# arkworks-rs/ripp

Measured on AMD Instinct MI355X. Metric: SIPP prover pairing-products/sec at n=2^20 BLS12-381, higher is better.
Workload: dtype u32

## Files before the change

### ripp_amd/csrc/bls12_381/tower.hpp

```cpp
#pragma once
#include "fp.hpp"
#include "fp_inv.hpp"

namespace ripp {

struct Fp2 {
    Fp c0, c1;
    RIPP_HD static Fp2 zero() { return {Fp::zero(), Fp::zero()}; }
    RIPP_HD static Fp2 one() { return {Fp::one(), Fp::zero()}; }
    RIPP_HD bool is_zero() const { return c0.is_zero() && c1.is_zero(); }
    RIPP_HD bool operator==(const Fp2& o) const { return c0 == o.c0 && c1 == o.c1; }
};
RIPP_HD Fp2 add(const Fp2& a, const Fp2& b) { return {add(a.c0, b.c0), add(a.c1, b.c1)}; }
RIPP_HD Fp2 sub(const Fp2& a, const Fp2& b) { return {sub(a.c0, b.c0), sub(a.c1, b.c1)}; }
RIPP_HD Fp2 neg(const Fp2& a) { return {neg(a.c0), neg(a.c1)}; }
RIPP_HD Fp2 dbl(const Fp2& a) { return {dbl(a.c0), dbl(a.c1)}; }
RIPP_HD Fp2 conj(const Fp2& a) { return {a.c0, neg(a.c1)}; }
#if defined(RIPP_BLS12_377)
RIPP_HD Fp mul5(const Fp& a) { const Fp t = dbl(dbl(a)); return add(t, a); }
RIPP_MID Fp2 mul(const Fp2& a, const Fp2& b) {
    const Fp t0 = fmul(a.c0, b.c0), t1 = fmul(a.c1, b.c1);
    const Fp m = fmul(add(a.c0, a.c1), add(b.c0, b.c1));
    return {sub(t0, mul5(t1)), sub(sub(m, t0), t1)};
}
RIPP_MID Fp2 sqr(const Fp2& a) {
    const Fp m = fmul(a.c0, a.c1);
    return {add(fmul(add(a.c0, a.c1), sub(a.c0, mul5(a.c1))), dbl(dbl(m))), dbl(m)};
}
RIPP_MID Fp2 mul_fp(const Fp2& a, const Fp& s) { return {fmul(a.c0, s), fmul(a.c1, s)}; }
RIPP_HD Fp2 mul_xi(const Fp2& a) { return {neg(mul5(a.c1)), a.c0}; }
RIPP_MID Fp2 inv(const Fp2& a) {
    const Fp n = finv(add(fsqr(a.c0), mul5(fsqr(a.c1))));
    return {fmul(a.c0, n), neg(fmul(a.c1, n))};
}
#else
RIPP_MID Fp2 mul(const Fp2& a, const Fp2& b) {
    const Fp t0 = fmul(a.c0, b.c0), t1 = fmul(a.c1, b.c1);
    const Fp m = fmul(add(a.c0, a.c1), add(b.c0, b.c1));
    return {sub(t0, t1), sub(sub(m, t0), t1)};
}
RIPP_MID Fp2 sqr(const Fp2& a) {
    const Fp m = fmul(a.c0, a.c1);
    return {fmul(add(a.c0, a.c1), sub(a.c0, a.c1)), dbl(m)};
}
RIPP_MID Fp2 mul_fp(const Fp2& a, const Fp& s) { return {fmul(a.c0, s), fmul(a.c1, s)}; }
RIPP_HD Fp2 mul_xi(const Fp2& a) { return {sub(a.c0, a.c1), add(a.c0, a.c1)}; }
RIPP_MID Fp2 inv(const Fp2& a) {
    const Fp n = finv(add(fsqr(a.c0), fsqr(a.c1)));
    return {fmul(a.c0, n), neg(fmul(a.c1, n))};
}
#endif

RIPP_HD Fp2 finv(const Fp2& a) { return inv(a); }
#if defined(__HIP_DEVICE_COMPILE__) && !defined(RIPP_NO_FP2_LAZY) && defined(RIPP_BLS12_377)
RIPP_MID Fp2 fmul(const Fp2& a, const Fp2& b) { return {fmul2_add(a.c0, b.c0, neg(mul5(a.c1)), b.c1), fmul2_add(a.c0, b.c1, a.c1, b.c0)}; }
#elif defined(__HIP_DEVICE_COMPILE__) && !defined(RIPP_NO_FP2_LAZY)
RIPP_MID Fp2 fmul(const Fp2& a, const Fp2& b) { return {fmul2_add(a.c0, b.c0, neg(a.c1), b.c1), fmul2_add(a.c0, b.c1, a.c1, b.c0)}; }
#else
RIPP_HD Fp2 fmul(const Fp2& a, const Fp2& b) { return mul(a, b); }
#endif
RIPP_HD Fp2 fsqr(const Fp2& a) { return sqr(a); }

struct Fp6 {
    Fp2 c0, c1, c2;
    RIPP_HD static Fp6 zero() { return {Fp2::zero(), Fp2::zero(), Fp2::zero()}; }
    RIPP_HD static Fp6 one() { return {Fp2::one(), Fp2::zero(), Fp2::zero()}; }
    RIPP_HD bool operator==(const Fp6& o) const { return c0 == o.c0 && c1 == o.c1 && c2 == o.c2; }
};
RIPP_HD Fp6 add(const Fp6& a, const Fp6& b) { return {add(a.c0, b.c0), add(a.c1, b.c1), add(a.c2, b.c2)}; }
RIPP_HD Fp6 sub(const Fp6& a, const Fp6& b) { return {sub(a.c0, b.c0), sub(a.c1, b.c1), sub(a.c2, b.c2)}; }
RIPP_HD Fp6 neg(const Fp6& a) { return {neg(a.c0), neg(a.c1), neg(a.c2)}; }
RIPP_HD Fp6 mul_v(const Fp6& a) { return {mul_xi(a.c2), a.c0, a.c1}; }
RIPP_MID Fp6 mul(const Fp6& a, const Fp6& b) {
    const Fp2 v0 = mul(a.c0, b.c0), v1 = mul(a.c1, b.c1), v2 = mul(a.c2, b.c2);
    const Fp2 t0 = add(mul_xi(sub(sub(mul(add(a.c1, a.c2), add(b.c1, b.c2)), v1), v2)), v0);
    const Fp2 t1 = add(sub(sub(mul(add(a.c0, a.c1), add(b.c0, b.c1)), v0), v1), mul_xi(v2));
    const Fp2 t2 = add(sub(sub(mul(add(a.c0, a.c2), add(b.c0, b.c2)), v0), v2), v1);
    return {t0, t1, t2};
}
RIPP_MID Fp6 mul_by_01(const Fp6& a, const Fp2& b0, const Fp2& b1) {
    const Fp2 v0 = mul(a.c0, b0), v1 = mul(a.c1, b1);
    const Fp2 t0 = add(mul_xi(sub(mul(add(a.c1, a.c2), b1), v1)), v0);
    const Fp2 t1 = sub(sub(mul(add(a.c0, a.c1), add(b0, b1)), v0), v1);
    const Fp2 t2 = add(sub(mul(add(a.c0, a.c2), b0), v0), v1);
    return {t0, t1, t2};
}
RIPP_MID Fp6 mul_by_1(const Fp6& a, const Fp2& b1) { return {mul_xi(mul(a.c2, b1)), mul(a.c0, b1), mul(a.c1, b1)}; }
RIPP_FN Fp6 inv(const Fp6& a) {
    const Fp2 A = sub(sqr(a.c0), mul_xi(mul(a.c1, a.c2)));
    const Fp2 B = sub(mul_xi(sqr(a.c2)), mul(a.c0, a.c1));
    const Fp2 C = sub(sqr(a.c1), mul(a.c0, a.c2));
    const Fp2 F = inv(add(mul_xi(add(mul(a.c2, B), mul(a.c1, C))), mul(a.c0, A)));
    return {mul(A, F), mul(B, F), mul(C, F)};
}

struct Fp12 {
    Fp6 c0, c1;
    RIPP_HD static Fp12 one() { return {Fp6::one(), Fp6::zero()}; }
    RIPP_HD bool operator==(const Fp12& o) const { return c0 == o.c0 && c1 == o.c1; }
};
RIPP_HD Fp12 conj(const Fp12& a) { return {a.c0, neg(a.c1)}; }
RIPP_MID Fp12 mul(const Fp12& a, const Fp12& b) {
    const Fp6 v0 = mul(a.c0, b.c0), v1 = mul(a.c1, b.c1);
    const Fp6 x = sub(sub(mul(add(a.c0, a.c1), add(b.c0, b.c1)), v0), v1);
    return {add(v0, mul_v(v1)), x};
}
RIPP_MID Fp12 sqr(const Fp12& a) {
    const Fp6 v0 = mul(a.c0, a.c1);
    const Fp6 s = sub(sub(mul(add(a.c0, a.c1), add(a.c0, mul_v(a.c1))), v0), mul_v(v0));
    return {s, add(v0, v0)};
}
RIPP_MID Fp12 mul_by_014(const Fp12& f, const Fp2& c0, const Fp2& c1, const Fp2& c4) {
    const Fp6 aa = mul_by_01(f.c0, c0, c1);
    const Fp6 bb = mul_by_1(f.c1, c4);
    const Fp6 s = sub(sub(mul_by_01(add(f.c1, f.c0), c0, add(c1, c4)), aa), bb);
    return {add(mul_v(bb), aa), s};
}
RIPP_MID Fp12 mul_by_034(const Fp12& f, const Fp2& c0, const Fp2& d0, const Fp2& d1) {
    const Fp6 a = {mul(f.c0.c0, c0), mul(f.c0.c1, c0), mul(f.c0.c2, c0)};
    const Fp6 b = mul_by_01(f.c1, d0, d1);
    const Fp6 e = sub(sub(mul_by_01(add(f.c0, f.c1), add(c0, d0), d1), a), b);
    return {add(a, mul_v(b)), e};
}
RIPP_FN Fp12 inv(const Fp12& a) {
    const Fp6 t = inv(sub(mul(a.c0, a.c0), mul_v(mul(a.c1, a.c1))));
    return {mul(a.c0, t), neg(mul(a.c1, t))};
}

RIPP_FN Fp12 frobenius(const Fp12& a, int k) {
    Fp2 g[6] = {a.c0.c0, a.c1.c0, a.c0.c1, a.c1.c1, a.c0.c2, a.c1.c2};
    for (int i = 0; i < 6; ++i) {
        constexpr uint32_t T[3][6][2][12] = {
            {{RIPP_FROB1_W0_C0, RIPP_FROB1_W0_C1}, {RIPP_FROB1_W1_C0, RIPP_FROB1_W1_C1}, {RIPP_FROB1_W2_C0, RIPP_FROB1_W2_C1},
             {RIPP_FROB1_W3_C0, RIPP_FROB1_W3_C1}, {RIPP_FROB1_W4_C0, RIPP_FROB1_W4_C1}, {RIPP_FROB1_W5_C0, RIPP_FROB1_W5_C1}},
            {{RIPP_FROB2_W0_C0, RIPP_FROB2_W0_C1}, {RIPP_FROB2_W1_C0, RIPP_FROB2_W1_C1}, {RIPP_FROB2_W2_C0, RIPP_FROB2_W2_C1},
             {RIPP_FROB2_W3_C0, RIPP_FROB2_W3_C1}, {RIPP_FROB2_W4_C0, RIPP_FROB2_W4_C1}, {RIPP_FROB2_W5_C0, RIPP_FROB2_W5_C1}},
            {{RIPP_FROB3_W0_C0, RIPP_FROB3_W0_C1}, {RIPP_FROB3_W1_C0, RIPP_FROB3_W1_C1}, {RIPP_FROB3_W2_C0, RIPP_FROB3_W2_C1},
             {RIPP_FROB3_W3_C0, RIPP_FROB3_W3_C1}, {RIPP_FROB3_W4_C0, RIPP_FROB3_W4_C1}, {RIPP_FROB3_W5_C0, RIPP_FROB3_W5_C1}}};
        Fp2 coef;
        for (int j = 0; j < 12; ++j) { coef.c0.l[j] = T[k - 1][i][0][j]; coef.c1.l[j] = T[k - 1][i][1][j]; }
        g[i] = mul((k & 1) ? conj(g[i]) : g[i], coef);
    }
    return {{g[0], g[2], g[4]}, {g[1], g[3], g[5]}};
}

RIPP_HD void fp4_sqr(Fp2& o0, Fp2& o1, const Fp2& x, const Fp2& y) {
    const Fp2 t0 = sqr(x), t1 = sqr(y);
    o1 = sub(sub(sqr(add(x, y)), t0), t1);
    o0 = add(t0, mul_xi(t1));
}
RIPP_FN Fp12 cyclotomic_sqr(const Fp12& a) {
    const Fp2 &z0 = a.c0.c0, &z4 = a.c0.c1, &z3 = a.c0.c2, &z2 = a.c1.c0, &z1 = a.c1.c1, &z5 = a.c1.c2;
    Fp2 t0, t1, t2, t3, t4, t5;
    fp4_sqr(t0, t1, z0, z1); fp4_sqr(t2, t3, z2, z3); fp4_sqr(t4, t5, z4, z5);
    const Fp2 xt5 = mul_xi(t5);
    Fp12 o;
    o.c0.c0 = add(dbl(sub(t0, z0)), t0);
    o.c1.c1 = add(dbl(add(t1, z1)), t1);
    o.c1.c0 = add(dbl(add(xt5, z2)), xt5);
    o.c0.c2 = add(dbl(sub(t4, z3)), t4);
    o.c0.c1 = add(dbl(sub(t2, z4)), t2);
    o.c1.c2 = add(dbl(add(t3, z5)), t3);
    return o;
}

}
```

### ripp_amd/csrc/engine.hip

```cpp
#include <hip/hip_runtime.h>
#include <atomic>
#include <csignal>
#include <sched.h>
#include <condition_variable>
#include <deque>
#include <functional>
#include <memory>
#include <future>
#include <chrono>
#include <cmath>
#include <cstdio>
#include <cstring>
#include <cstdlib>
#include <mutex>
#include <string>
#include <thread>
#include <vector>
#ifndef RIPP_BUILD_STAMP
#define RIPP_BUILD_STAMP __DATE__ " " __TIME__
#endif
#include "../../include/ripp_hip.h"
#include "recode.hpp"
#include "kernels.hpp"
#include "line_products.hpp"
#include "msm.hpp"
#include "scale.hpp"
#include "vm.hpp"
#include "fq_curve.hpp"
#include "fq_curve2.hpp"
#include "fq_validate.hpp"
#include "fq_line_products.hpp"
#include "fq_line_products_k.hpp"
#include "fq_miller.hpp"
#include "fq_scale.hpp"
#include "fq_msm.hpp"
#include "msm_batch.hpp"
#include "tpc.hpp"
#include "gipa_mexp.hpp"
#include "tipa_scalar.hpp"
#include "vm_fold2.hpp"
#include "host_fs.hpp"
#include "wire.hpp"
#include "config.hpp"

using namespace ripp;

static_assert(sizeof(ripp_fp) == sizeof(Fp) && sizeof(ripp_fr) == sizeof(Fr), "limb layout");
static_assert(sizeof(ripp_gt) == sizeof(Fp12) && sizeof(ripp_g1a) == sizeof(G1A) && sizeof(ripp_g2a) == sizeof(G2A), "layout");
static_assert(sizeof(ripp_g1j) == sizeof(G1J) && sizeof(ripp_g2j) == sizeof(G2J), "layout");

namespace {

std::mutex g_mu;
ripp_config g_cfg{}; bool g_cfg_set = false;
thread_local std::string g_err;

#if defined(__HIP_DEVICE_COMPILE__)
#define RIPP_CPU_RELAX() ((void)0)
#else
#define RIPP_CPU_RELAX() __builtin_ia32_pause()
#endif
class HostPool {
public:
    explicit HostPool(unsigned n) { for (unsigned i = 0; i < n; ++i) th_.emplace_back([this]() { run(); }); }
    ~HostPool() { { std::lock_guard<std::mutex> lk(mu_); stop_ = true; } cv_.notify_all(); for (auto& t : th_) t.join(); }
    unsigned size() const { return (unsigned)th_.size(); }
// ... 2307 lines not shown
```

### ripp_amd/csrc/tipa_api.inc

```
extern "C++" {
struct FoldPre { DevBuf pow_h, parts; bool ready = false; void release() { pow_h.release(); parts.release(); } };
struct VecBufCache { std::vector<DevBuf> bufs; bool full = false;
    void adopt(const std::vector<DevBuf*>& l) { if (!full || bufs.size() != l.size()) return; size_t i = 0; for (DevBuf* b : l) std::swap(*b, bufs[i++]); full = false; }
    void park(const std::vector<DevBuf*>& l) { (void)hipDeviceSynchronize(); if (full) { for (DevBuf* b : l) b->release(); return; } bufs.resize(l.size()); size_t i = 0; for (DevBuf* b : l) { bufs[i].release(); std::swap(*b, bufs[i++]); } full = true; }
    void release() { for (DevBuf& b : bufs) b.release(); full = false; } };
static VecBufCache g_tipp_cache, g_ssm_cache, g_mexp_cache, g_scal_cache;
struct VecLease { VecBufCache* cache; std::vector<DevBuf*> bufs;
    VecLease(VecBufCache* c, std::initializer_list<DevBuf*> l) : cache(c), bufs(l) { if (cache) cache->adopt(bufs); }
    ~VecLease() { if (cache) cache->park(bufs); else { (void)hipDeviceSynchronize(); for (DevBuf* b : bufs) b->release(); } }
    VecLease(const VecLease&) = delete; VecLease& operator=(const VecLease&) = delete; };
static FoldPre g_tpc_pre;
static void vec_caches_release() { g_tipp_cache.release(); g_ssm_cache.release(); g_mexp_cache.release(); g_scal_cache.release(); g_tpc_pre.release(); }
template <class F> static int32_t fold_precompute(Engine* e, hipStream_t st, const Affine<F>* hi, size_t half, FoldPre& fp) {
    fp.ready = false;
    if (half == 0 || half > e->cfg.pub.vm_fold_max || e->cfg.pub.no_vm || e->cfg.pub.no_precompute) return RIPP_OK;
    constexpr bool g1 = std::is_same<F, Fp>::value;
    int32_t rc; if ((rc = fp.pow_h.reserve(half * sizeof(Jac<F>))) || (rc = fp.parts.reserve((g1 ? 4 : 8) * half * sizeof(Jac<F>)))) return rc;
    hipLaunchKernelGGL(HIP_KERNEL_NAME(k_vm_pow2<F>), dim3(nblk(half, 4 * VM_EPW)), dim3(256), 4 * VM_EPW * VmCurve<F>::SLOTS * sizeof(VmSlot), st, hi, (uint32_t)half, g1 ? 64 : 32, fp.pow_h.as<Jac<F>>());
    HIPCHK(hipGetLastError());
    fp.ready = true; return RIPP_OK;
}
template <class F> struct FoldReq { const Affine<F>* hi; const Affine<F>* lo; Affine<F>* out; Fr s; FoldPre* fp; };
static bool fold_batching(const Engine* e, size_t half) { return half != 0 && half <= e->cfg.pub.vm_fold_max && !e->cfg.pub.no_vm && !e->cfg.pub.no_precompute; }
template <class F> static int32_t fold_precompute_batch(Engine* e, hipStream_t st, FoldReq<F>* req, int cnt, size_t half) {
// ... 60 lines not shown
    if (half <= e->cfg.pub.vm_fold_max && !e->cfg.pub.no_vm) {
        hipLaunchKernelGGL(k_vm_fold_g2_split, dim3(nblk(half, 4 * VM_EPW), 4), dim3(256), 4 * VM_EPW * VM_G2_SLOTS * sizeof(VmSlot), st, hi, (uint32_t)half, gls_digits(s), qt.as<G2J>(), e->vm_flag.as<uint32_t>());
        hipLaunchKernelGGL(k_vm_combine_g2, dim3(nblk(half, 4 * VM_EPW)), dim3(256), 4 * VM_EPW * VM_G2_SLOTS * sizeof(VmSlot), st, qt.as<G2J>(), lo, (uint32_t)half, jac.as<G2J>());
    } else if (half <= e->cfg.pub.gls_split_max) {
        if (!e->cfg.pub.no_fq) {
            uint8_t* flags = qt.as<uint8_t>() + qt_bytes;
            hipLaunchKernelGGL(k_fold_g2_gls_split_q, dim3(nblk(half, 64), 4), dim3(64), 0, st, hi, (uint32_t)half, gls_digits(s), qt.as<G2J>(), flags);
#if !defined(RIPP_INLINE_FALLBACK)
            hipLaunchKernelGGL(k_fold_g2_gls_split_fix, dim3(FIX_GRID), dim3(64), 0, st, hi, (uint32_t)half, gls_digits(s), qt.as<G2J>(), flags);
#endif
        } else
        hipLaunchKernelGGL(k_fold_g2_gls_split, dim3(nblk(half, 64), 4), dim3(64), 0, st, hi, (uint32_t)half, gls_digits(s), qt.as<G2J>());
        hipLaunchKernelGGL(k_fold_g2_combine, dim3(nblk(half, 64)), dim3(64), 0, st, qt.as<G2J>(), lo, (uint32_t)half, jac.as<G2J>());
    } else if (fold_g2_table_pays(e, half)) {
        if ((rc = fold_g2_table(e, st, hi, lo, half, s, jac))) return rc;
    } else {
        hipLaunchKernelGGL(k_fold_g2_gls, dim3(nblk(half, 64)), dim3(64), 0, st, hi, lo, (uint32_t)half, gls_digits(s), qt.as<uint4>(), qstride, jac.as<G2J>());
    }
    HIPCHK(hipGetLastError());
    return e->normalize_dev<Fp2>(jac.as<G2J>(), half, out, st);
}
}

extern "C++" { static Fp12 gt_pow_host(const Fp12& x, const Fr& k); }

extern "C++" {
static Fp12 gt_pow_gls_strings(const Fp12& z, const GlsDigits& g, unsigned strings) {
    Fp12 b[4], bi[4];
    b[0] = z;
    for (int j = 1; j < 4; ++j) if ((strings >> j) & 1u) { b[j] = frobenius(z, j); if (BLS_X_NEG && (j & 1)) b[j] = conj(b[j]); }
    for (int j = 0; j < 4; ++j) if ((strings >> j) & 1u) bi[j] = conj(b[j]);
    Fp12 acc = Fp12::one(); bool st = false;
    for (int pos = g.len - 1; pos >= 0; --pos) {
        if (st) acc = cyclotomic_sqr(acc);
        for (int j = 0; j < 4; ++j) {
            if (!((strings >> j) & 1u)) continue;
            const int d = g.d[j][pos];
            if (d != 0) { const Fp12& m = d > 0 ? b[j] : bi[j]; acc = st ? mul(acc, m) : m; st = true; }
        }
    }
    return acc;
}
static Fp12 gt_pow_gls(const Fp12& z, const Fr& k) { return gt_pow_gls_strings(z, gls_digits(k), 15u); }
}

struct TippVecs {
    DevBuf A, A2, KB, KB2, B, B2, KA, KA2, jac1, jac1b, jac2, jac2b, qt2;
    DevBuf AU, AU2, jac1u;
    FoldPre pA, pKB, pB, pKA, pAU;
    VecLease lease;
    explicit TippVecs(bool use_cache = true)
        : lease(use_cache ? &g_tipp_cache : nullptr, {&A, &A2, &KB, &KB2, &B, &B2, &KA, &KA2, &jac1, &jac1b, &jac2, &jac2b, &qt2, &AU, &AU2, &jac1u, &pA.pow_h, &pA.parts, &pKB.pow_h, &pKB.parts,
                                                       &pB.pow_h, &pB.parts, &pKA.pow_h, &pKA.parts, &pAU.pow_h, &pAU.parts}) {}
    int32_t reserve(size_t n) {
        int32_t rc;
        for (DevBuf* b : {&A, &A2, &KB, &KB2}) if ((rc = b->reserve(n * sizeof(G1A)))) return rc;
        for (DevBuf* b : {&B, &B2, &KA, &KA2}) if ((rc = b->reserve(n * sizeof(G2A)))) return rc;
        if ((rc = jac1.reserve(n * sizeof(G1J))) || (rc = jac2.reserve(n * sizeof(G2J)))) return rc;
        return RIPP_OK;
    }
};

extern "C++" {
template <class Launch> static int32_t fork_join_folds(Engine* e, Launch&& launch) {
    int32_t rc;
    HIPCHK(hipEventRecord(e->ev_fork, e->stream));
    for (hipStream_t st : {e->stream2, e->stream3, e->stream4, e->stream5}) HIPCHK(hipStreamWaitEvent(st, e->ev_fork, 0));
// ... 578 lines not shown
API int32_t ripp_aggregate_proofs(const ripp_srs* srs, const ripp_g1a* a, const ripp_g2a* b, const ripp_g1a* c, size_t n, ripp_aggregate_proof* out, ripp_stats* st) {
    if (n < 2 || (n & (n - 1))) return RIPP_ERR_POW2;
    LOCK; ENGINE;
    if (!srs || !a || !b || !c || !out || !out->ab_com_steps || !out->ab_transcript || !out->c_com_gt || !out->c_com_g1 || !out->c_transcript) return RIPP_ERR_ARG;
    return aggregate_impl(e, srs, a, b, c, n, out, st, ShardCtx());
}
API int32_t ripp_aggregate_proofs_sharded(const ripp_srs* srs, const ripp_g1a* a, const ripp_g2a* b, const ripp_g1a* c, size_t n_local, ripp_aggregate_proof* out, ripp_stats* st) {
    if (n_local == 0 || (n_local & (n_local - 1))) return RIPP_ERR_POW2;
    LOCK; ENGINE;
    comm_mark_proof();
    if (!srs || !a || !b || !c || !out || !out->ab_com_steps || !out->ab_transcript || !out->c_com_gt || !out->c_com_g1 || !out->c_transcript) return RIPP_ERR_ARG;
    const ShardCtx sc = ShardCtx::from_comm();
    if (sc.world & (sc.world - 1)) { set_err("the number of ranks must be a power of two"); return RIPP_ERR_POW2; }
    if (n_local * (size_t)sc.world < 2) return RIPP_ERR_POW2;
    return aggregate_impl(e, srs, a, b, c, n_local, out, st, sc);
}

extern "C++" {
static bool gt_in_cyclotomic(const Fp12& x) {
    const Fp2* c[6] = {&x.c0.c0, &x.c0.c1, &x.c0.c2, &x.c1.c0, &x.c1.c1, &x.c1.c2};
    bool zero = true; for (const Fp2* v : c) zero = zero && v->c0.is_zero() && v->c1.is_zero();
    return !zero && mul(frobenius(frobenius(x, 2), 2), x) == frobenius(x, 2);
}
static Fp12 gt_pow_host(const Fp12& x, const Fr& k) {
    const Fr c = from_mont(k);
    int8_t d[260]; const int len = naf_recode(c.l, 8, d, 258);
    const Fp12 xi = conj(x);
    Fp12 acc = Fp12::one(); bool st = false;
    for (int i = len - 1; i >= 0; --i) {
        if (st) acc = cyclotomic_sqr(acc);
        if (d[i] != 0) { const Fp12& m = d[i] > 0 ? x : xi; acc = st ? mul(acc, m) : m; st = true; }
    }
    return acc;
}
template <class F> static Jac<F> smul_host(const Affine<F>& p, const Fr& k) { const Fr c = from_mont(k); return scalar_mul_bits(p, c.l, 255); }
template <class F> static Jac<F> load_jac(const void* p) { Jac<F> r; std::memcpy(&r, p, sizeof r); return r; }
static Fp12 load_gt(const ripp_gt* p) { Fp12 r; std::memcpy(&r, p, sizeof r); return r; }
static Fr load_fr(const ripp_fr* p) { Fr r; std::memcpy(&r, p, sizeof r); return r; }

static int32_t pairing_host_pts(Engine* e, const std::vector<G1A>& a, const std::vector<G2A>& b, Fp12* out) {
    G1A* da; G2A* db; int32_t rc; ripp_gt z;
    if ((rc = upload<G1A>(e, e->tmpA, a.data(), a.size(), &da)) || (rc = upload<G2A>(e, e->tmpB, b.data(), b.size(), &db))) return rc;
    if ((rc = pairing_product_dev(e, da, db, a.size(), &z))) return rc;
    std::memcpy(out, &z, sizeof z); return RIPP_OK;
}
static int32_t pairing_eq(Engine* e, const G1J& a1, const G2J& b1, const G1J& a2, const G2J& b2, bool* ok) {
    Fp12 z; int32_t rc = pairing_host_pts(e, {to_affine(a1), neg(to_affine(a2))}, {to_affine(b1), to_affine(b2)}, &z); if (rc) return rc;
    *ok = (z == Fp12::one()); return RIPP_OK;
}
static Fr ck_poly_eval(const std::vector<Fr>& tr, const Fr& z, const Fr& r_shift) {
    Fr p = mul(mul(z, z), r_shift), acc = Fr::one();
    for (const Fr& x : tr) { acc = mul(acc, add(Fr::one(), mul(x, p))); p = mul(p, p); }
    return acc;
}
struct VSrs { G1J g, g_beta; G2J h, h_alpha; };
static VSrs load_vsrs(const ripp_verifier_srs* v) { return {load_jac<Fp>(&v->g), load_jac<Fp>(&v->g_beta), load_jac<Fp2>(&v->h), load_jac<Fp2>(&v->h_alpha)}; }
static int32_t kzg_verify_g2(Engine* e, const VSrs& v, const G2J& ck_final, const G2J& opening, const std::vector<Fr>& tr, const Fr& r_shift, const Fr& c, bool* ok) {
// ... 175 lines not shown
```

Baseline: 2.632 million.

## Add 64-bit lazy-reduction host tower arithmetic for CPU-side Fp2/Fp6/Fp12 ops

```diff
diff --git a/ripp_amd/csrc/bls12_381/host_tower.hpp b/ripp_amd/csrc/bls12_381/host_tower.hpp
--- /dev/null
+++ b/ripp_amd/csrc/bls12_381/host_tower.hpp
@@ -0,0 +1,408 @@
+#pragma once
+#if !defined(__HIP_DEVICE_COMPILE__)
+#include <stdint.h>
+#include <stdlib.h>
+#include <stdio.h>
+#include "fp.hpp"
+#if defined(__x86_64__) && !defined(RIPP_HT_PORTABLE)
+#include <immintrin.h>
+#define RIPP_HT_X86 1
+#endif
+
+namespace ripp {
+namespace ht {
+
+typedef unsigned __int128 u128;
+#define RIPP_HT inline __attribute__((always_inline))
+#if !defined(RIPP_HT_LEAF)
+#define RIPP_HT_LEAF inline __attribute__((noinline))
+#endif
+
+using P = FpParams;
+constexpr int M = P::N / 2;
+static_assert(M == 6, "384-bit container");
+constexpr uint64_t pl(int i) { return (uint64_t)P::mod(2 * i) | ((uint64_t)P::mod(2 * i + 1) << 32); }
+constexpr uint64_t inv64() { const uint64_t x = P::INV; return x * (2 + pl(0) * x); }
+constexpr uint64_t INV64 = inv64();
+static_assert((uint64_t)(INV64 * pl(0)) == ~0ull, "-p^-1 mod 2^64");
+
+constexpr int LIM(int m) { return m <= 0 ? 0 : (int)((((u128)(unsigned)m) << 64) / ((u128)pl(M - 1) + 1)); }
+static_assert(P::BITS >= 377 && P::BITS <= 383 && (pl(M - 1) >> (P::BITS - 321)) == 1, "p has BITS bits");
+static_assert(LIM(1) >= (1 << (383 - P::BITS)), "2^384 / p from BITS");
+constexpr bool fits(int A, int B, int n) { return A >= 0 && B >= 0 && B <= n && A <= LIM(n - B); }
+constexpr bool wide_cap(int A, int B) { return A >= 0 && B >= 0 && B < LIM(1) && A <= (LIM(1) - B) * LIM(1); }
+
+struct L6 { uint64_t l[6]; };
+struct L12 { uint64_t l[12]; };
+constexpr L6 kp(int k) {
+    L6 r{}; uint64_t c = 0;
+    for (int i = 0; i < 6; ++i) { const u128 z = (u128)pl(i) * (unsigned)k + c; r.l[i] = (uint64_t)z; c = (uint64_t)(z >> 64); }
+    return r;
+}
+constexpr L12 woff(int A, int B) {
+    L12 s{};
+    for (int i = 0; i < 6; ++i) {
+        uint64_t c = 0;
+        for (int j = 0; j < 6; ++j) { const u128 z = (u128)pl(i) * pl(j) + s.l[i + j] + c; s.l[i + j] = (uint64_t)z; c = (uint64_t)(z >> 64); }
+        s.l[i + 6] = c;
+    }
+    L12 r{}; uint64_t c = 0;
+    for (int i = 0; i < 12; ++i) { const u128 z = (u128)s.l[i] * (unsigned)A + c; r.l[i] = (uint64_t)z; c = (uint64_t)(z >> 64); }
+    const L6 q = kp(B); c = 0;
+    for (int i = 0; i < 6; ++i) { const u128 z = (u128)r.l[6 + i] + q.l[i] + c; r.l[6 + i] = (uint64_t)z; c = (uint64_t)(z >> 64); }
+    return r;
+}
+
+template <int K> struct Nr { static_assert(K >= 1 && K <= LIM(1), "narrow value must stay below 2^384"); uint64_t l[6]; };
+template <int A, int B = 0> struct Wd { static_assert(wide_cap(A, B), "wide value must stay below 2^768"); uint64_t l[12]; };
+using H1 = Nr<1>;
+
+#if defined(RIPP_HT_CHECK)
+[[noreturn]] inline void ht_fail(const char* what) { fprintf(stderr, "host_tower bound violated: %s\n", what); abort(); }
+template <int N> inline bool lt_limbs(const uint64_t* a, const uint64_t* b) { for (int i = N - 1; i >= 0; --i) { if (a[i] != b[i]) return a[i] < b[i]; } return false; }
+template <int K> RIPP_HT void chk(const Nr<K>& a, const char* w) { constexpr L6 b = kp(K); if (lt_limbs<6>(b.l, a.l)) ht_fail(w); }
+template <int A, int B> RIPP_HT void chk(const Wd<A, B>& a, const char* w) { constexpr L12 b = woff(A, B); if (lt_limbs<12>(b.l, a.l)) ht_fail(w); }
+#define RIPP_HT_ASSERT(c, w) do { if (!(c)) ht_fail(w); } while (0)
+#else
+template <class T> RIPP_HT void chk(const T&, const char*) {}
+#define RIPP_HT_ASSERT(c, w) do { } while (0)
+#endif
+
+#if defined(RIPP_HT_X86)
+typedef unsigned long long ull;
+RIPP_HT uint8_t adc(uint8_t c, uint64_t a, uint64_t b, uint64_t& o) { ull r; c = _addcarry_u64(c, a, b, &r); o = r; return c; }
+RIPP_HT uint8_t sbb(uint8_t c, uint64_t a, uint64_t b, uint64_t& o) { ull r; c = _subborrow_u64(c, a, b, &r); o = r; return c; }
+#else
+RIPP_HT uint8_t adc(uint8_t c, uint64_t a, uint64_t b, uint64_t& o) { const u128 z = (u128)a + b + c; o = (uint64_t)z; return (uint8_t)(z >> 64); }
+RIPP_HT uint8_t sbb(uint8_t c, uint64_t a, uint64_t b, uint64_t& o) { const u128 z = (u128)a - b - c; o = (uint64_t)z; return (uint8_t)((z >> 64) & 1); }
+#endif
+
+RIPP_HT void rowmul(uint64_t* r, uint64_t x, const uint64_t* y) {
+    uint64_t lo[6], hi[6];
+#pragma unroll
+    for (int j = 0; j < 6; ++j) { const u128 z = (u128)x * y[j]; lo[j] = (uint64_t)z; hi[j] = (uint64_t)(z >> 64); }
+    r[0] = lo[0]; uint8_t c = 0;
+#pragma unroll
+    for (int j = 1; j < 6; ++j) c = adc(c, lo[j], hi[j - 1], r[j]);
+    (void)adc(c, hi[5], 0, r[6]);
+}
+RIPP_HT void mulw(uint64_t* __restrict t, const uint64_t* a, const uint64_t* b) {
+    uint64_t al[6], bl[6], w[12];
+#pragma unroll
+    for (int i = 0; i < 6; ++i) { al[i] = a[i]; bl[i] = b[i]; }
+    rowmul(w, al[0], bl);
+#pragma unroll
+    for (int i = 1; i < 6; ++i) {
+        uint64_t r[7]; rowmul(r, al[i], bl);
+        uint8_t c = 0;
+#pragma unroll
+        for (int j = 0; j < 6; ++j) c = adc(c, w[i + j], r[j], w[i + j]);
+        (void)adc(c, r[6], 0, w[i + 6]);
+    }
+#pragma unroll
+    for (int i = 0; i < 12; ++i) t[i] = w[i];
+}
+RIPP_HT void sqrw(uint64_t* __restrict t, const uint64_t* a) {
+    uint64_t al[6], w[12];
+#pragma unroll
+    for (int i = 0; i < 6; ++i) al[i] = a[i];
+    w[0] = 0;
+    { uint64_t c = 0;
+#pragma unroll
+      for (int j = 1; j < 6; ++j) { const u128 z = (u128)al[0] * al[j] + c; w[j] = (uint64_t)z; c = (uint64_t)(z >> 64); }
+      w[6] = c; }
+#pragma unroll
+    for (int i = 1; i < 5; ++i) {
+        uint64_t c = 0;
+#pragma unroll
+        for (int j = i + 1; j < 6; ++j) { const u128 z = (u128)al[i] * al[j] + w[i + j] + c; w[i + j] = (uint64_t)z; c = (uint64_t)(z >> 64); }
+        w[i + 6] = c;
+    }
+    w[11] = w[10] >> 63;
+#pragma unroll
+    for (int i = 10; i >= 2; --i) w[i] = (w[i] << 1) | (w[i - 1] >> 63);
+    w[1] <<= 1;
+    uint8_t c = 0;
+#pragma unroll
+    for (int i = 0; i < 6; ++i) {
+        const u128 d = (u128)al[i] * al[i];
+        c = adc(c, w[2 * i], (uint64_t)d, w[2 * i]);
+        c = adc(c, w[2 * i + 1], (uint64_t)(d >> 64), w[2 * i + 1]);
+    }
+#pragma unroll
+    for (int i = 0; i < 12; ++i) t[i] = w[i];
+}
+RIPP_HT void csub_p(uint64_t* r) {
+    uint64_t d[6]; uint8_t bo = 0;
+#pragma unroll
+    for (int i = 0; i < 6; ++i) bo = sbb(bo, r[i], pl(i), d[i]);
+#pragma unroll
+    for (int i = 0; i < 6; ++i) r[i] = bo ? r[i] : d[i];
+}
+template <int NCS>
+RIPP_HT_LEAF void redc_raw(uint64_t* r, const uint64_t* tin) {
+    uint64_t t[12], pm[6];
+#pragma unroll
+    for (int i = 0; i < 12; ++i) t[i] = tin[i];
+#pragma unroll
+    for (int j = 0; j < 6; ++j) pm[j] = pl(j);
+    uint8_t k = 0;
+#pragma unroll
+    for (int i = 0; i < 6; ++i) {
+        uint64_t q[7]; rowmul(q, t[i] * INV64, pm);
+        uint8_t c = 0;
+#pragma unroll
+        for (int j = 0; j < 6; ++j) c = adc(c, t[i + j], q[j], t[i + j]);
+        c = adc(c, t[i + 6], q[6], t[i + 6]);
+        uint8_t c2 = adc(k, t[i + 6], 0, t[i + 6]);
+        k = (uint8_t)(c + c2);
+        RIPP_HT_ASSERT(k <= 1, "redc carry pair");
+    }
+    RIPP_HT_ASSERT(k == 0, "redc carry");
+#pragma unroll
+    for (int i = 0; i < 6; ++i) r[i] = t[i + 6];
+    csub_p(r);
+    if (NCS > 1) csub_p(r);
+}
+
+template <int A, int B> RIPP_HT Nr<A + B> nadd(const Nr<A>& a, const Nr<B>& b) {
+    Nr<A + B> r; uint8_t c = 0;
+#pragma unroll
+    for (int i = 0; i < 6; ++i) c = adc(c, a.l[i], b.l[i], r.l[i]);
+    RIPP_HT_ASSERT(c == 0, "nadd carry"); chk(r, "nadd");
+    return r;
+}
+template <int A, int B> RIPP_HT Nr<A + B> nsub(const Nr<A>& a, const Nr<B>& b) {
+    constexpr L6 off = kp(B);
+    Nr<A + B> r; uint8_t c = 0;
+#pragma unroll
+    for (int i = 0; i < 6; ++i) c = adc(c, a.l[i], off.l[i], r.l[i]);
+    RIPP_HT_ASSERT(c == 0, "nsub carry");
+    uint8_t bo = 0;
+#pragma unroll
+    for (int i = 0; i < 6; ++i) bo = sbb(bo, r.l[i], b.l[i], r.l[i]);
+    RIPP_HT_ASSERT(bo == 0, "nsub borrow"); chk(r, "nsub");
+    return r;
+}
+RIPP_HT H1 madd(const H1& a, const H1& b) {
+    H1 r; uint8_t c = 0;
+#pragma unroll
+    for (int i = 0; i < 6; ++i) c = adc(c, a.l[i], b.l[i], r.l[i]);
+    csub_p(r.l);
+    return r;
+}
+RIPP_HT H1 msub(const H1& a, const H1& b) {
+    H1 r; uint8_t bo = 0;
+#pragma unroll
+    for (int i = 0; i < 6; ++i) bo = sbb(bo, a.l[i], b.l[i], r.l[i]);
+    const uint64_t mask = 0ull - (uint64_t)bo; uint8_t c = 0;
+#pragma unroll
+    for (int i = 0; i < 6; ++i) c = adc(c, r.l[i], pl(i) & mask, r.l[i]);
+    return r;
+}
+RIPP_HT H1 mdbl(const H1& a) { return madd(a, a); }
+RIPP_HT H1 mneg(const H1& a) { H1 z; for (int i = 0; i < 6; ++i) z.l[i] = 0; return msub(z, a); }
+RIPP_HT H1 mmul5(const H1& a) { return madd(mdbl(mdbl(a)), a); }
+
+template <int A, int B> RIPP_HT Wd<A * B> mul_wide(const Nr<A>& a, const Nr<B>& b) { Wd<A * B> r; mulw(r.l, a.l, b.l); chk(r, "mul_wide"); return r; }
+template <int A> RIPP_HT Wd<A * A> sqr_wide(const Nr<A>& a) { Wd<A * A> r; sqrw(r.l, a.l); chk(r, "sqr_wide"); return r; }
+template <int A, int B, int C, int D> RIPP_HT Wd<A + C, B + D> wadd(const Wd<A, B>& a, const Wd<C, D>& b) {
+    Wd<A + C, B + D> r; uint8_t c = 0;
+#pragma unroll
+    for (int i = 0; i < 12; ++i) c = adc(c, a.l[i], b.l[i], r.l[i]);
+    RIPP_HT_ASSERT(c == 0, "wadd carry"); chk(r, "wadd");
+    return r;
+}
+template <int A, int B, int C, int D> RIPP_HT Wd<A + C, B + D> wsub(const Wd<A, B>& a, const Wd<C, D>& b) {
+    constexpr L12 off = woff(C, D);
+    Wd<A + C, B + D> r; uint8_t c = 0;
+#pragma unroll
+    for (int i = (C == 0 ? 6 : 0); i < 12; ++i) c = adc(c, a.l[i], off.l[i], r.l[i]);
+    if (C == 0) { for (int i = 0; i < 6; ++i) r.l[i] = a.l[i]; }
+    RIPP_HT_ASSERT(c == 0, "wsub carry");
+    uint8_t bo = 0;
+#pragma unroll
+    for (int i = 0; i < 12; ++i) bo = sbb(bo, r.l[i], b.l[i], r.l[i]);
+    RIPP_HT_ASSERT(bo == 0, "wsub borrow"); chk(r, "wsub");
+    return r;
+}
+template <int R, int A, int C> RIPP_HT Wd<R> wsub_nn(const Wd<A, 0>& a, const Wd<C, 0>& b) {
+    Wd<R> r; uint8_t bo = 0;
+#pragma unroll
+    for (int i = 0; i < 12; ++i) bo = sbb(bo, a.l[i], b.l[i], r.l[i]);
+    RIPP_HT_ASSERT(bo == 0, "wsub_nn borrow"); chk(r, "wsub_nn");
+    return r;
+}
+template <int A, int B> RIPP_HT Wd<5 * A, 5 * B> wmul5(const Wd<A, B>& a) { const auto a2 = wadd(a, a); return wadd(wadd(a2, a2), a); }
+template <int A, int B> RIPP_HT Wd<0, 1> fold(const Wd<A, B>& a) {
+    static_assert(fits(A, B, 2), "fold needs T <= 2 p 2^384");
+    Wd<0, 1> r;
+#pragma unroll
+    for (int i = 0; i < 12; ++i) r.l[i] = a.l[i];
+    csub_p(r.l + 6);
+    chk(r, "fold");
+    return r;
+}
+template <int A, int B> RIPP_HT auto r1(const Wd<A, B>& a) { if constexpr (fits(A, B, 1)) return a; else return fold(a); }
+template <class X, class Y> RIPP_HT auto sadd(const X& a, const Y& b) { return wadd(r1(a), r1(b)); }
+template <class X, class Y> RIPP_HT auto ssub(const X& a, const Y& b) { return wsub(r1(a), r1(b)); }
+template <int A, int B> RIPP_HT H1 redc(const Wd<A, B>& a) {
+    static_assert(fits(A, B, 2), "the reduction needs T <= 2 p 2^384");
+    H1 r;
+    redc_raw<fits(A, B, 1) ? 1 : 2>(r.l, a.l);
+    chk(r, "redc");
+    return r;
+}
+
+RIPP_HT H1 fp_mul(const H1& a, const H1& b) { return redc(mul_wide(a, b)); }
+RIPP_HT H1 fp_sqr(const H1& a) { return redc(sqr_wide(a)); }
+RIPP_HT bool fp_is_zero(const H1& a) { uint64_t o = 0; for (int i = 0; i < 6; ++i) o |= a.l[i]; return o == 0; }
+RIPP_HT_LEAF H1 fp_inv(const H1& a) {
+    H1 r = a; bool started = false;
+    for (int i = P::N * 32 - 1; i >= 0; --i) {
+        if (started) r = fp_sqr(r);
+        if ((P::pm2(i >> 5) >> (i & 31)) & 1u) { if (started) r = fp_mul(r, a); started = true; }
+    }
+    return r;
+}
+
+#if defined(RIPP_BLS12_377)
+constexpr int NR = 5;
+#else
+constexpr int NR = 1;
+#endif
+template <int K> struct N2 { Nr<K> c0, c1; };
+template <class X, class Y> struct W2 { X c0; Y c1; };
+template <class X, class Y> RIPP_HT W2<X, Y> mk2(const X& x, const Y& y) { return {x, y}; }
+using H2 = N2<1>;
+struct H6 { H2 c0, c1, c2; };
+struct H12 { H6 c0, c1; };
+
+template <int A, int B> RIPP_HT N2<A + B> n2add(const N2<A>& a, const N2<B>& b) { return {nadd(a.c0, b.c0), nadd(a.c1, b.c1)}; }
+RIPP_HT H2 m2add(const H2& a, const H2& b) { return {madd(a.c0, b.c0), madd(a.c1, b.c1)}; }
+RIPP_HT H2 m2sub(const H2& a, const H2& b) { return {msub(a.c0, b.c0), msub(a.c1, b.c1)}; }
+RIPP_HT H2 m2dbl(const H2& a) { return {mdbl(a.c0), mdbl(a.c1)}; }
+#if defined(RIPP_BLS12_377)
+RIPP_HT H2 m2xi(const H2& a) { return {mneg(mmul5(a.c1)), a.c0}; }
+#else
+RIPP_HT H2 m2xi(const H2& a) { return {msub(a.c0, a.c1), madd(a.c0, a.c1)}; }
+#endif
+RIPP_HT H6 m6add(const H6& a, const H6& b) { return {m2add(a.c0, b.c0), m2add(a.c1, b.c1), m2add(a.c2, b.c2)}; }
+RIPP_HT H6 m6mulv(const H6& a) { return {m2xi(a.c2), a.c0, a.c1}; }
+
+template <class X, class Y> RIPP_HT auto w2add(const X& a, const Y& b) { return mk2(sadd(a.c0, b.c0), sadd(a.c1, b.c1)); }
+template <class X, class Y> RIPP_HT auto w2sub(const X& a, const Y& b) { return mk2(ssub(a.c0, b.c0), ssub(a.c1, b.c1)); }
+template <class X> RIPP_HT auto w2xi(const X& a) {
+#if defined(RIPP_BLS12_377)
+    const Wd<0, 0> z{};
+    return mk2(ssub(z, wmul5(r1(a.c1))), a.c0);
+#else
+    return mk2(ssub(a.c0, a.c1), sadd(a.c0, a.c1));
+#endif
+}
+template <class X> RIPP_HT H2 redc2(const X& a) { return {redc(a.c0), redc(a.c1)}; }
+
+template <int A, int B> RIPP_HT_LEAF auto mul2w(const N2<A>& a, const N2<B>& b) {
+    const auto t0 = mul_wide(a.c0, b.c0), t1 = mul_wide(a.c1, b.c1);
+    const auto t2 = mul_wide(nadd(a.c0, a.c1), nadd(b.c0, b.c1));
+    const auto c1 = wsub_nn<2 * A * B>(wsub_nn<3 * A * B>(t2, t0), t1);
+#if defined(RIPP_BLS12_377)
+    const auto c0 = wsub(t0, wmul5(t1));
+#else
+    const auto c0 = wsub(t0, t1);
+#endif
+    return mk2(c0, c1);
+}
+RIPP_HT_LEAF auto sqr2w(const H2& a) {
+#if defined(RIPP_BLS12_377)
+    const auto m = mul_wide(a.c0, a.c1);
+    const auto a15 = nadd(nadd(nadd(a.c1, a.c1), nadd(a.c1, a.c1)), a.c1);
+    const auto m2 = wadd(m, m);
+    return mk2(wadd(mul_wide(nadd(a.c0, a.c1), nsub(a.c0, a15)), wadd(m2, m2)), m2);
+#else
+    return mk2(mul_wide(nadd(a.c0, a.c1), nsub(a.c0, a.c1)), mul_wide(nadd(a.c0, a.c0), a.c1));
+#endif
+}
+RIPP_HT H2 fp2_mul(const H2& a, const H2& b) { return redc2(mul2w(a, b)); }
+RIPP_HT H2 fp2_sqr(const H2& a) { return redc2(sqr2w(a)); }
+
+template <class T0, class T1, class T2> struct W6 { T0 c0; T1 c1; T2 c2; };
+template <class T0, class T1, class T2> RIPP_HT W6<T0, T1, T2> mk6(const T0& a, const T1& b, const T2& c) { return {a, b, c}; }
+template <class X, class V, class W> RIPP_HT auto kar2(const X& x, const V& v, const W& w) {
+    return mk2(wsub_nn<2 + 2 * NR>(wsub_nn<3 + 3 * NR>(x.c0, v.c0), w.c0), wsub_nn<4>(wsub_nn<6>(x.c1, v.c1), w.c1));
+}
+template <class X, class V> RIPP_HT auto kar1(const X& x, const V& v) { return mk2(wsub_nn<1 + NR>(x.c0, v.c0), wsub_nn<2>(x.c1, v.c1)); }
+
+RIPP_HT auto mul6w(const H6& a, const H6& b) {
+    const auto v0 = mul2w(a.c0, b.c0), v1 = mul2w(a.c1, b.c1), v2 = mul2w(a.c2, b.c2);
+    const auto d12 = kar2(mul2w(n2add(a.c1, a.c2), n2add(b.c1, b.c2)), v1, v2);
+    const auto d01 = kar2(mul2w(n2add(a.c0, a.c1), n2add(b.c0, b.c1)), v0, v1);
+    const auto d02 = kar2(mul2w(n2add(a.c0, a.c2), n2add(b.c0, b.c2)), v0, v2);
+    return mk6(w2add(w2xi(d12), v0), w2add(d01, w2xi(v2)), w2add(d02, v1));
+}
+RIPP_HT auto mul6w_01(const H6& a, const H2& b0, const H2& b1) {
+    const auto v0 = mul2w(a.c0, b0), v1 = mul2w(a.c1, b1);
+    const auto d1 = kar1(mul2w(n2add(a.c1, a.c2), b1), v1);
+    const auto d01 = kar2(mul2w(n2add(a.c0, a.c1), n2add(b0, b1)), v0, v1);
+    const auto d2 = kar1(mul2w(n2add(a.c0, a.c2), b0), v0);
+    return mk6(w2add(w2xi(d1), v0), d01, w2add(d2, v1));
+}
+RIPP_HT auto mul6w_1(const H6& a, const H2& b1) { return mk6(w2xi(mul2w(a.c2, b1)), mul2w(a.c0, b1), mul2w(a.c1, b1)); }
+RIPP_HT auto mul6w_0(const H6& a, const H2& b0) { return mk6(mul2w(a.c0, b0), mul2w(a.c1, b0), mul2w(a.c2, b0)); }
+
+template <class X, class Y> RIPP_HT auto w6add(const X& a, const Y& b) { return mk6(w2add(a.c0, b.c0), w2add(a.c1, b.c1), w2add(a.c2, b.c2)); }
+template <class X, class Y> RIPP_HT auto w6sub(const X& a, const Y& b) { return mk6(w2sub(a.c0, b.c0), w2sub(a.c1, b.c1), w2sub(a.c2, b.c2)); }
+template <class X> RIPP_HT auto w6mulv(const X& a) { return mk6(w2xi(a.c2), a.c0, a.c1); }
+template <class X> RIPP_HT H6 redc6(const X& a) { return {redc2(a.c0), redc2(a.c1), redc2(a.c2)}; }
+
+RIPP_HT H6 fp6_mul(const H6& a, const H6& b) { return redc6(mul6w(a, b)); }
+RIPP_HT H6 fp6_mul_by_01(const H6& a, const H2& b0, const H2& b1) { return redc6(mul6w_01(a, b0, b1)); }
+RIPP_HT H6 fp6_mul_by_1(const H6& a, const H2& b1) { return redc6(mul6w_1(a, b1)); }
+
+RIPP_HT H12 fp12_mul(const H12& a, const H12& b) {
+    const auto v0 = mul6w(a.c0, b.c0), v1 = mul6w(a.c1, b.c1);
+    const auto x = mul6w(m6add(a.c0, a.c1), m6add(b.c0, b.c1));
+    return {redc6(w6add(v0, w6mulv(v1))), redc6(w6sub(w6sub(x, v0), v1))};
+}
+RIPP_HT H12 fp12_sqr(const H12& a) {
+    const auto v = mul6w(a.c0, a.c1);
+    const auto x = mul6w(m6add(a.c0, a.c1), m6add(a.c0, m6mulv(a.c1)));
+    const H6 h = redc6(v);
+    return {redc6(w6sub(w6sub(x, v), w6mulv(v))), {m2dbl(h.c0), m2dbl(h.c1), m2dbl(h.c2)}};
+}
+RIPP_HT H12 fp12_mul_by_014(const H12& f, const H2& c0, const H2& c1, const H2& c4) {
+    const auto aa = mul6w_01(f.c0, c0, c1);
+    const auto bb = mul6w_1(f.c1, c4);
+    const auto s = mul6w_01(m6add(f.c1, f.c0), c0, m2add(c1, c4));
+    return {redc6(w6add(w6mulv(bb), aa)), redc6(w6sub(w6sub(s, aa), bb))};
+}
+RIPP_HT H12 fp12_mul_by_034(const H12& f, const H2& c0, const H2& d0, const H2& d1) {
+    const auto a = mul6w_0(f.c0, c0);
+    const auto b = mul6w_01(f.c1, d0, d1);
+    const auto e = mul6w_01(m6add(f.c0, f.c1), m2add(c0, d0), d1);
+    return {redc6(w6add(a, w6mulv(b))), redc6(w6sub(w6sub(e, a), b))};
+}
+
+RIPP_HT void fp4_sqr(H2& o0, H2& o1, const H2& x, const H2& y) {
+    const auto t0 = sqr2w(x), t1 = sqr2w(y), s = sqr2w(m2add(x, y));
+    o1 = redc2(w2sub(w2sub(s, t0), t1));
+    o0 = redc2(w2add(t0, w2xi(t1)));
+}
+RIPP_HT H12 cyclotomic_sqr(const H12& a) {
+    const H2 &z0 = a.c0.c0, &z4 = a.c0.c1, &z3 = a.c0.c2, &z2 = a.c1.c0, &z1 = a.c1.c1, &z5 = a.c1.c2;
+    H2 t0, t1, t2, t3, t4, t5;
+    fp4_sqr(t0, t1, z0, z1); fp4_sqr(t2, t3, z2, z3); fp4_sqr(t4, t5, z4, z5);
+    const H2 xt5 = m2xi(t5);
+    H12 o;
+    o.c0.c0 = m2add(m2dbl(m2sub(t0, z0)), t0);
+    o.c1.c1 = m2add(m2dbl(m2add(t1, z1)), t1);
+    o.c1.c0 = m2add(m2dbl(m2add(xt5, z2)), xt5);
+    o.c0.c2 = m2add(m2dbl(m2sub(t4, z3)), t4);
+    o.c0.c1 = m2add(m2dbl(m2sub(t2, z4)), t2);
+    o.c1.c2 = m2add(m2dbl(m2add(t3, z5)), t3);
+    return o;
+}
+
+}
+}
+#endif
diff --git a/ripp_amd/csrc/bls12_381/tower.hpp b/ripp_amd/csrc/bls12_381/tower.hpp
--- a/ripp_amd/csrc/bls12_381/tower.hpp
+++ b/ripp_amd/csrc/bls12_381/tower.hpp
@@ -1,6 +1,10 @@
 #pragma once
 #include "fp.hpp"
 #include "fp_inv.hpp"
+#if !defined(__HIP_DEVICE_COMPILE__) && !defined(RIPP_HOST_TOWER_REF)
+#include "host_tower.hpp"
+#define RIPP_HOST_TOWER 1
+#endif
 
 namespace ripp {
 
@@ -11,6 +15,15 @@
     RIPP_HD bool is_zero() const { return c0.is_zero() && c1.is_zero(); }
     RIPP_HD bool operator==(const Fp2& o) const { return c0 == o.c0 && c1 == o.c1; }
 };
+#if defined(RIPP_HOST_TOWER)
+static_assert(sizeof(ht::H1) == sizeof(Fp) && sizeof(ht::H2) == sizeof(Fp2), "the host forms read the same image");
+template <class To, class From> RIPP_HD To hcast(const From& a) { static_assert(sizeof(To) == sizeof(From), "layout"); return __builtin_bit_cast(To, a); }
+#endif
+#if defined(RIPP_HOST_TOWER)
+RIPP_HD Fp tinv(const Fp& a) { return hcast<Fp>(ht::fp_inv(hcast<ht::H1>(a))); }
+#else
+RIPP_HD Fp tinv(const Fp& a) { return finv(a); }
+#endif
 RIPP_HD Fp2 add(const Fp2& a, const Fp2& b) { return {add(a.c0, b.c0), add(a.c1, b.c1)}; }
 RIPP_HD Fp2 sub(const Fp2& a, const Fp2& b) { return {sub(a.c0, b.c0), sub(a.c1, b.c1)}; }
 RIPP_HD Fp2 neg(const Fp2& a) { return {neg(a.c0), neg(a.c1)}; }
@@ -19,34 +32,46 @@
 #if defined(RIPP_BLS12_377)
 RIPP_HD Fp mul5(const Fp& a) { const Fp t = dbl(dbl(a)); return add(t, a); }
 RIPP_MID Fp2 mul(const Fp2& a, const Fp2& b) {
+#if defined(RIPP_HOST_TOWER)
+    return hcast<Fp2>(ht::fp2_mul(hcast<ht::H2>(a), hcast<ht::H2>(b)));
+#endif
     const Fp t0 = fmul(a.c0, b.c0), t1 = fmul(a.c1, b.c1);
     const Fp m = fmul(add(a.c0, a.c1), add(b.c0, b.c1));
     return {sub(t0, mul5(t1)), sub(sub(m, t0), t1)};
 }
 RIPP_MID Fp2 sqr(const Fp2& a) {
+#if defined(RIPP_HOST_TOWER)
+    return hcast<Fp2>(ht::fp2_sqr(hcast<ht::H2>(a)));
+#endif
     const Fp m = fmul(a.c0, a.c1);
     return {add(fmul(add(a.c0, a.c1), sub(a.c0, mul5(a.c1))), dbl(dbl(m))), dbl(m)};
 }
 RIPP_MID Fp2 mul_fp(const Fp2& a, const Fp& s) { return {fmul(a.c0, s), fmul(a.c1, s)}; }
 RIPP_HD Fp2 mul_xi(const Fp2& a) { return {neg(mul5(a.c1)), a.c0}; }
 RIPP_MID Fp2 inv(const Fp2& a) {
-    const Fp n = finv(add(fsqr(a.c0), mul5(fsqr(a.c1))));
+    const Fp n = tinv(add(fsqr(a.c0), mul5(fsqr(a.c1))));
     return {fmul(a.c0, n), neg(fmul(a.c1, n))};
 }
 #else
 RIPP_MID Fp2 mul(const Fp2& a, const Fp2& b) {
+#if defined(RIPP_HOST_TOWER)
+    return hcast<Fp2>(ht::fp2_mul(hcast<ht::H2>(a), hcast<ht::H2>(b)));
+#endif
     const Fp t0 = fmul(a.c0, b.c0), t1 = fmul(a.c1, b.c1);
     const Fp m = fmul(add(a.c0, a.c1), add(b.c0, b.c1));
     return {sub(t0, t1), sub(sub(m, t0), t1)};
 }
 RIPP_MID Fp2 sqr(const Fp2& a) {
+#if defined(RIPP_HOST_TOWER)
+    return hcast<Fp2>(ht::fp2_sqr(hcast<ht::H2>(a)));
+#endif
     const Fp m = fmul(a.c0, a.c1);
     return {fmul(add(a.c0, a.c1), sub(a.c0, a.c1)), dbl(m)};
 }
 RIPP_MID Fp2 mul_fp(const Fp2& a, const Fp& s) { return {fmul(a.c0, s), fmul(a.c1, s)}; }
 RIPP_HD Fp2 mul_xi(const Fp2& a) { return {sub(a.c0, a.c1), add(a.c0, a.c1)}; }
 RIPP_MID Fp2 inv(const Fp2& a) {
-    const Fp n = finv(add(fsqr(a.c0), fsqr(a.c1)));
+    const Fp n = tinv(add(fsqr(a.c0), fsqr(a.c1)));
     return {fmul(a.c0, n), neg(fmul(a.c1, n))};
 }
 #endif
@@ -72,6 +97,9 @@
 RIPP_HD Fp6 neg(const Fp6& a) { return {neg(a.c0), neg(a.c1), neg(a.c2)}; }
 RIPP_HD Fp6 mul_v(const Fp6& a) { return {mul_xi(a.c2), a.c0, a.c1}; }
 RIPP_MID Fp6 mul(const Fp6& a, const Fp6& b) {
+#if defined(RIPP_HOST_TOWER)
+    return hcast<Fp6>(ht::fp6_mul(hcast<ht::H6>(a), hcast<ht::H6>(b)));
+#endif
     const Fp2 v0 = mul(a.c0, b.c0), v1 = mul(a.c1, b.c1), v2 = mul(a.c2, b.c2);
     const Fp2 t0 = add(mul_xi(sub(sub(mul(add(a.c1, a.c2), add(b.c1, b.c2)), v1), v2)), v0);
     const Fp2 t1 = add(sub(sub(mul(add(a.c0, a.c1), add(b.c0, b.c1)), v0), v1), mul_xi(v2));
@@ -79,13 +107,21 @@
     return {t0, t1, t2};
 }
 RIPP_MID Fp6 mul_by_01(const Fp6& a, const Fp2& b0, const Fp2& b1) {
+#if defined(RIPP_HOST_TOWER)
+    return hcast<Fp6>(ht::fp6_mul_by_01(hcast<ht::H6>(a), hcast<ht::H2>(b0), hcast<ht::H2>(b1)));
+#endif
     const Fp2 v0 = mul(a.c0, b0), v1 = mul(a.c1, b1);
     const Fp2 t0 = add(mul_xi(sub(mul(add(a.c1, a.c2), b1), v1)), v0);
     const Fp2 t1 = sub(sub(mul(add(a.c0, a.c1), add(b0, b1)), v0), v1);
     const Fp2 t2 = add(sub(mul(add(a.c0, a.c2), b0), v0), v1);
     return {t0, t1, t2};
 }
-RIPP_MID Fp6 mul_by_1(const Fp6& a, const Fp2& b1) { return {mul_xi(mul(a.c2, b1)), mul(a.c0, b1), mul(a.c1, b1)}; }
+RIPP_MID Fp6 mul_by_1(const Fp6& a, const Fp2& b1) {
+#if defined(RIPP_HOST_TOWER)
+    return hcast<Fp6>(ht::fp6_mul_by_1(hcast<ht::H6>(a), hcast<ht::H2>(b1)));
+#endif
+    return {mul_xi(mul(a.c2, b1)), mul(a.c0, b1), mul(a.c1, b1)};
+}
 RIPP_FN Fp6 inv(const Fp6& a) {
     const Fp2 A = sub(sqr(a.c0), mul_xi(mul(a.c1, a.c2)));
     const Fp2 B = sub(mul_xi(sqr(a.c2)), mul(a.c0, a.c1));
@@ -101,22 +137,34 @@
 };
 RIPP_HD Fp12 conj(const Fp12& a) { return {a.c0, neg(a.c1)}; }
 RIPP_MID Fp12 mul(const Fp12& a, const Fp12& b) {
+#if defined(RIPP_HOST_TOWER)
+    return hcast<Fp12>(ht::fp12_mul(hcast<ht::H12>(a), hcast<ht::H12>(b)));
+#endif
     const Fp6 v0 = mul(a.c0, b.c0), v1 = mul(a.c1, b.c1);
     const Fp6 x = sub(sub(mul(add(a.c0, a.c1), add(b.c0, b.c1)), v0), v1);
     return {add(v0, mul_v(v1)), x};
 }
 RIPP_MID Fp12 sqr(const Fp12& a) {
+#if defined(RIPP_HOST_TOWER)
+    return hcast<Fp12>(ht::fp12_sqr(hcast<ht::H12>(a)));
+#endif
     const Fp6 v0 = mul(a.c0, a.c1);
     const Fp6 s = sub(sub(mul(add(a.c0, a.c1), add(a.c0, mul_v(a.c1))), v0), mul_v(v0));
     return {s, add(v0, v0)};
 }
 RIPP_MID Fp12 mul_by_014(const Fp12& f, const Fp2& c0, const Fp2& c1, const Fp2& c4) {
+#if defined(RIPP_HOST_TOWER)
+    return hcast<Fp12>(ht::fp12_mul_by_014(hcast<ht::H12>(f), hcast<ht::H2>(c0), hcast<ht::H2>(c1), hcast<ht::H2>(c4)));
+#endif
     const Fp6 aa = mul_by_01(f.c0, c0, c1);
     const Fp6 bb = mul_by_1(f.c1, c4);
     const Fp6 s = sub(sub(mul_by_01(add(f.c1, f.c0), c0, add(c1, c4)), aa), bb);
     return {add(mul_v(bb), aa), s};
 }
 RIPP_MID Fp12 mul_by_034(const Fp12& f, const Fp2& c0, const Fp2& d0, const Fp2& d1) {
+#if defined(RIPP_HOST_TOWER)
+    return hcast<Fp12>(ht::fp12_mul_by_034(hcast<ht::H12>(f), hcast<ht::H2>(c0), hcast<ht::H2>(d0), hcast<ht::H2>(d1)));
+#endif
     const Fp6 a = {mul(f.c0.c0, c0), mul(f.c0.c1, c0), mul(f.c0.c2, c0)};
     const Fp6 b = mul_by_01(f.c1, d0, d1);
     const Fp6 e = sub(sub(mul_by_01(add(f.c0, f.c1), add(c0, d0), d1), a), b);
@@ -145,11 +193,17 @@
 }
 
 RIPP_HD void fp4_sqr(Fp2& o0, Fp2& o1, const Fp2& x, const Fp2& y) {
+#if defined(RIPP_HOST_TOWER)
+    { ht::H2 h0, h1; ht::fp4_sqr(h0, h1, hcast<ht::H2>(x), hcast<ht::H2>(y)); o0 = hcast<Fp2>(h0); o1 = hcast<Fp2>(h1); return; }
+#endif
     const Fp2 t0 = sqr(x), t1 = sqr(y);
     o1 = sub(sub(sqr(add(x, y)), t0), t1);
     o0 = add(t0, mul_xi(t1));
 }
 RIPP_FN Fp12 cyclotomic_sqr(const Fp12& a) {
+#if defined(RIPP_HOST_TOWER)
+    return hcast<Fp12>(ht::cyclotomic_sqr(hcast<ht::H12>(a)));
+#endif
     const Fp2 &z0 = a.c0.c0, &z4 = a.c0.c1, &z3 = a.c0.c2, &z2 = a.c1.c0, &z1 = a.c1.c1, &z5 = a.c1.c2;
     Fp2 t0, t1, t2, t3, t4, t5;
     fp4_sqr(t0, t1, z0, z1); fp4_sqr(t2, t3, z2, z3); fp4_sqr(t4, t5, z4, z5);
diff --git a/ripp_amd/csrc/engine.hip b/ripp_amd/csrc/engine.hip
--- a/ripp_amd/csrc/engine.hip
+++ b/ripp_amd/csrc/engine.hip
@@ -42,6 +42,7 @@
 #include "host_fs.hpp"
 #include "wire.hpp"
 #include "config.hpp"
+#include "gt_pow.hpp"
 
 using namespace ripp;
 
diff --git a/ripp_amd/csrc/gt_pow.hpp b/ripp_amd/csrc/gt_pow.hpp
--- /dev/null
+++ b/ripp_amd/csrc/gt_pow.hpp
@@ -0,0 +1,37 @@
+#pragma once
+#include "recode.hpp"
+#include "bls12_381/pairing.hpp"
+
+namespace ripp {
+
+inline Fp12 gt_pow_gls_strings(const Fp12& z, const GlsDigits& g, unsigned strings) {
+    Fp12 b[4], bi[4];
+    b[0] = z;
+    for (int j = 1; j < 4; ++j) if ((strings >> j) & 1u) { b[j] = frobenius(z, j); if (BLS_X_NEG && (j & 1)) b[j] = conj(b[j]); }
+    for (int j = 0; j < 4; ++j) if ((strings >> j) & 1u) bi[j] = conj(b[j]);
+    Fp12 acc = Fp12::one(); bool st = false;
+    for (int pos = g.len - 1; pos >= 0; --pos) {
+        if (st) acc = cyclotomic_sqr(acc);
+        for (int j = 0; j < 4; ++j) {
+            if (!((strings >> j) & 1u)) continue;
+            const int d = g.d[j][pos];
+            if (d != 0) { const Fp12& m = d > 0 ? b[j] : bi[j]; acc = st ? mul(acc, m) : m; st = true; }
+        }
+    }
+    return acc;
+}
+inline Fp12 gt_pow_gls(const Fp12& z, const Fr& k) { return gt_pow_gls_strings(z, gls_digits(k), 15u); }
+
+inline Fp12 gt_pow_host(const Fp12& x, const Fr& k) {
+    const Fr c = from_mont(k);
+    int8_t d[260]; const int len = naf_recode(c.l, 8, d, 258);
+    const Fp12 xi = conj(x);
+    Fp12 acc = Fp12::one(); bool st = false;
+    for (int i = len - 1; i >= 0; --i) {
+        if (st) acc = cyclotomic_sqr(acc);
+        if (d[i] != 0) { const Fp12& m = d[i] > 0 ? x : xi; acc = st ? mul(acc, m) : m; st = true; }
+    }
+    return acc;
+}
+
+}
diff --git a/ripp_amd/csrc/tipa_api.inc b/ripp_amd/csrc/tipa_api.inc
--- a/ripp_amd/csrc/tipa_api.inc
+++ b/ripp_amd/csrc/tipa_api.inc
@@ -106,27 +106,6 @@
 }
 }
 
-extern "C++" { static Fp12 gt_pow_host(const Fp12& x, const Fr& k); }
-
-extern "C++" {
-static Fp12 gt_pow_gls_strings(const Fp12& z, const GlsDigits& g, unsigned strings) {
-    Fp12 b[4], bi[4];
-    b[0] = z;
-    for (int j = 1; j < 4; ++j) if ((strings >> j) & 1u) { b[j] = frobenius(z, j); if (BLS_X_NEG && (j & 1)) b[j] = conj(b[j]); }
-    for (int j = 0; j < 4; ++j) if ((strings >> j) & 1u) bi[j] = conj(b[j]);
-    Fp12 acc = Fp12::one(); bool st = false;
-    for (int pos = g.len - 1; pos >= 0; --pos) {
-        if (st) acc = cyclotomic_sqr(acc);
-        for (int j = 0; j < 4; ++j) {
-            if (!((strings >> j) & 1u)) continue;
-            const int d = g.d[j][pos];
-            if (d != 0) { const Fp12& m = d > 0 ? b[j] : bi[j]; acc = st ? mul(acc, m) : m; st = true; }
-        }
-    }
-    return acc;
-}
-static Fp12 gt_pow_gls(const Fp12& z, const Fr& k) { return gt_pow_gls_strings(z, gls_digits(k), 15u); }
-}
 
 struct TippVecs {
     DevBuf A, A2, KB, KB2, B, B2, KA, KA2, jac1, jac1b, jac2, jac2b, qt2;
@@ -751,17 +730,6 @@
     bool zero = true; for (const Fp2* v : c) zero = zero && v->c0.is_zero() && v->c1.is_zero();
     return !zero && mul(frobenius(frobenius(x, 2), 2), x) == frobenius(x, 2);
 }
-static Fp12 gt_pow_host(const Fp12& x, const Fr& k) {
-    const Fr c = from_mont(k);
-    int8_t d[260]; const int len = naf_recode(c.l, 8, d, 258);
-    const Fp12 xi = conj(x);
-    Fp12 acc = Fp12::one(); bool st = false;
-    for (int i = len - 1; i >= 0; --i) {
-        if (st) acc = cyclotomic_sqr(acc);
-        if (d[i] != 0) { const Fp12& m = d[i] > 0 ? x : xi; acc = st ? mul(acc, m) : m; st = true; }
-    }
-    return acc;
-}
 template <class F> static Jac<F> smul_host(const Affine<F>& p, const Fr& k) { const Fr c = from_mont(k); return scalar_mul_bits(p, c.l, 255); }
 template <class F> static Jac<F> load_jac(const void* p) { Jac<F> r; std::memcpy(&r, p, sizeof r); return r; }
 static Fp12 load_gt(const ripp_gt* p) { Fp12 r; std::memcpy(&r, p, sizeof r); return r; }
```

New measurement: 2.672 million (median of 5 runs). +1.5%, better.
